# matteosantama/dantzig

Measured on AMD Instinct MI355X. Metric: simplex_iterations_per_sec, higher is better.
Workload: dtype f64

## Files before the change

### dantzig_amd/_ffi.py

```python
from __future__ import annotations

import ctypes as C
import os

import numpy as np

_HERE = os.path.dirname(os.path.abspath(__file__))
LIB_PATH = os.path.join(_HERE, "libdantzig_amd.so")

OPTIMAL, UNBOUNDED, INFEASIBLE, ITER_LIMIT, SINGULAR, PANIC, RUNNING, NEAR_TIE, NODE_LIMIT = range(9)
E_DEVICE, E_ARG, E_NOMEM = -1, -2, -3
STRICT, FAST, AUTO = 0, 1, 2
PRICE_AUTO, PRICE_SEQ, PRICE_WAVE, PRICE_TREE = 0, 1, 2, 3
STEP_PRIMAL, STEP_DUAL = 0, 1
NEAR_TIE_COUNT, NEAR_TIE_STOP = 0, 1
(K_STATUS, K_FTRAN, K_RATIO, K_BTRAN, K_PRICE, K_UPDATE, K_BASIS_UPDATE, K_LU, K_XCHG1, K_XCHG2,
 K_COUNT) = range(11)
KERNEL_CLASSES = ["status", "ftran", "ratio", "btran", "price", "update", "basis_update", "lu",
                  "exchange1", "exchange2"]

EXPORTS = [
    "dzg_abi_version", "dzg_status_str", "dzg_last_error", "dzg_device_count",
    "dzg_opts_default", "dzg_solver_create", "dzg_solver_run", "dzg_solver_result",
    "dzg_solver_destroy", "dzg_core_solve", "dzg_model_solve", "dzg_build_standard_form",
    "dzg_kernel_lu_solve", "dzg_kernel_neg_t_dot", "dzg_kernel_first_pivot",
    "dzg_kernel_second_pivot", "dzg_gen_dense_lp", "dzg_gen_sparse_lp", "dzg_merge_candidates",
    "dzg_shard_record_doubles", "dzg_shard_phase1", "dzg_shard_phase2", "dzg_shard_phase3",
    "dzg_solver_poll", "dzg_solver_set_budget", "dzg_comm_unique_id", "dzg_shard_comm_init",
    "dzg_shard_run", "dzg_shard_run_lockstep", "dzg_solver_stream", "dzg_solver_refactor",
    "dzg_gen_dense_lp_block", "dzg_solver_set_profile", "dzg_kernel_neg_t_dot_csc",
    "dzg_shard_comm_size", "dzg_solver_upload_columns", "dzg_debug_hold_cus", "dzg_debug_hold_wait",
    "dzg_core_solve_full_csc", "dzg_debug_live_lists", "dzg_debug_rl_listed",
    "dzg_debug_basis_inverse", "dzg_batch_solve", "dzg_model_solve_batch", "dzg_mip_opts_default",
    "dzg_mip_solve", "dzg_mip_last_warm_stats", "dzg_debug_cand_reduce", "dzg_debug_chain_instance",
    "dzg_debug_chain_price_counts", "dzg_debug_wk_mismatch", "dzg_debug_chain_price_rule",
    "dzg_solver_duals", "dzg_batch_solve_duals", "dzg_model_solve_duals",
    "dzg_model_solve_batch_duals", "dzg_model_map_duals",
    "dzg_solver_ranging", "dzg_batch_solve_ranging", "dzg_model_solve_ranging",
    "dzg_model_solve_batch_ranging",
    "dzg_solver_ray", "dzg_batch_solve_rays", "dzg_model_solve_rays", "dzg_model_solve_batch_rays",
    "dzg_model_map_ray",
    "dzg_batch_solve_fast", "dzg_model_solve_batch_fast", "dzg_debug_batch_fast_inverse",
    "dzg_solver_reoptimize",
    "dzg_solver_extend", "dzg_solver_dims", "dzg_debug_matrix", "dzg_debug_matrix_rows",
    "dzg_debug_extend_ms",
    "dzg_solver_remove",
    "dzg_batch_solve_from", "dzg_debug_batch_restart_ms",
]

BATCH_MAX_ROWS = 128
DUALS_FRESH, DUALS_CARRIED = 1, 2
DUALS_SOURCE_NAMES = {DUALS_FRESH: "fresh", DUALS_CARRIED: "carried"}
RAY_PRIMAL, RAY_FARKAS = 1, 2


class Lp(C.Structure):
    _fields_ = [
        ("m", C.c_int64), ("n", C.c_int64), ("n_struct", C.c_int64),
        ("a", C.c_void_p), ("lda", C.c_int64), ("var_col", C.c_void_p),
        ("c", C.c_void_p), ("constant", C.c_double),
        ("basis", C.c_void_p), ("nonbasis", C.c_void_p), ("x", C.c_void_p), ("z", C.c_void_p),
        ("col_ptr", C.c_void_p), ("row_idx", C.c_void_p), ("val", C.c_void_p),
        ("xbar", C.c_void_p), ("zbar", C.c_void_p),
    ]


class Opts(C.Structure):
    _fields_ = [
        ("numerics", C.c_int32), ("price_kernel", C.c_int32), ("device", C.c_int32),
        ("auto_strict_rows", C.c_int32), ("max_iter", C.c_int64), ("epsilon", C.c_double),
        ("log_capacity", C.c_int64), ("poll_interval", C.c_int32), ("profile", C.c_int32),
        ("col_begin", C.c_int64), ("col_end", C.c_int64), ("rank", C.c_int32),
        ("world", C.c_int32), ("stream", C.c_void_p), ("refactor_interval", C.c_int64),
        ("a_is_block", C.c_int32), ("near_tie_action", C.c_int32),
        ("replicate_matrix", C.c_int32), ("auto_restart_rows", C.c_int32), ("tie_tol", C.c_double),
        ("seven_launches", C.c_int32), ("auto_strict_budget_s", C.c_int32),
        ("shard_rows", C.c_int32), ("reserved0", C.c_int32),
    ]


class Pivot(C.Structure):
    _fields_ = [("kind", C.c_int32), ("reserved", C.c_int32), ("entering", C.c_int64),
                ("leaving", C.c_int64), ("mu", C.c_double)]


class Result(C.Structure):
    _fields_ = [
        ("status", C.c_int32), ("numerics_used", C.c_int32), ("iterations", C.c_int64),
# ... 133 lines not shown
def lib() -> C.CDLL:
    global _lib
    if _lib is None:
        if not os.path.exists(LIB_PATH):
            raise DantzigAmdError(
                f"{LIB_PATH} is missing: build the HIP engine first "
                "(python -m dantzig_amd._build). dantzig_amd has no CPU fallback.")
        _lib = C.CDLL(LIB_PATH)
        _lib.dzg_status_str.restype = C.c_char_p
        _lib.dzg_last_error.restype = C.c_char_p
        _lib.dzg_merge_candidates.restype = C.c_int64
        _lib.dzg_solver_destroy.restype = None
        _lib.dzg_opts_default.restype = None
        _lib.dzg_gen_dense_lp.argtypes = [C.c_uint64, C.c_int64, C.c_int64, C.c_void_p, C.c_int64,
                                          C.c_void_p, C.c_void_p]
        _lib.dzg_gen_dense_lp_block.argtypes = [C.c_uint64, C.c_int64, C.c_int64, C.c_int64,
                                                C.c_int64, C.c_void_p, C.c_int64, C.c_void_p,
                                                C.c_void_p]
        _lib.dzg_solver_run.argtypes = [C.c_void_p, C.c_int64]
        _lib.dzg_solver_result.argtypes = [C.c_void_p, C.c_void_p]
        _lib.dzg_solver_destroy.argtypes = [C.c_void_p]
        _lib.dzg_shard_record_doubles.restype = C.c_int64
        _lib.dzg_shard_record_doubles.argtypes = [C.c_void_p]
        _lib.dzg_shard_phase1.argtypes = [C.c_void_p, C.c_void_p]
        _lib.dzg_shard_phase2.argtypes = [C.c_void_p, C.c_void_p, C.c_void_p]
        _lib.dzg_shard_phase3.argtypes = [C.c_void_p, C.c_void_p]
        _lib.dzg_solver_poll.argtypes = [C.c_void_p, C.c_void_p, C.c_void_p]
        _lib.dzg_solver_set_budget.argtypes = [C.c_void_p, C.c_int64]
        _lib.dzg_comm_unique_id.argtypes = [C.c_void_p]
        _lib.dzg_shard_comm_init.argtypes = [C.c_void_p, C.c_void_p]
        _lib.dzg_shard_run.argtypes = [C.c_void_p, C.c_int64]
        _lib.dzg_shard_comm_size.argtypes = [C.c_void_p]
        _lib.dzg_shard_run_lockstep.argtypes = [C.c_void_p, C.c_int32, C.c_int64]
        _lib.dzg_solver_stream.restype = C.c_void_p
        _lib.dzg_solver_stream.argtypes = [C.c_void_p]
        _lib.dzg_solver_refactor.argtypes = [C.c_void_p]
        _lib.dzg_solver_set_profile.argtypes = [C.c_void_p, C.c_int32]
        _lib.dzg_core_solve_full_csc.argtypes = [C.c_int64, C.c_int64, C.c_void_p, C.c_void_p,
                                                 C.c_void_p, C.c_void_p, C.c_double, C.c_void_p,
                                                 C.c_void_p, C.c_void_p, C.c_void_p, C.c_void_p,
                                                 C.c_void_p]
        _lib.dzg_debug_hold_cus.argtypes = [C.c_int32, C.c_int32, C.c_double]
        _lib.dzg_debug_live_lists.restype = C.c_int64
        _lib.dzg_debug_live_lists.argtypes = [C.c_void_p, C.c_void_p]
        _lib.dzg_debug_basis_inverse.restype = C.c_int
        _lib.dzg_debug_basis_inverse.argtypes = [C.c_void_p, C.c_int64, C.c_int64, C.c_void_p, C.c_void_p]
        _lib.dzg_debug_cand_reduce.restype = C.c_int
        _lib.dzg_debug_cand_reduce.argtypes = [C.c_int32, C.c_int32, C.c_int64, C.c_void_p, C.c_void_p,
                                               C.c_void_p, C.c_void_p, C.c_void_p, C.c_void_p, C.c_void_p]
        _lib.dzg_debug_chain_instance.restype = C.c_int
        _lib.dzg_debug_chain_instance.argtypes = [C.c_int32] * 7
        _lib.dzg_debug_chain_price_counts.argtypes = [C.c_void_p, C.c_void_p]
        _lib.dzg_debug_wk_mismatch.argtypes = [C.c_void_p, C.c_int32, C.c_void_p]
        _lib.dzg_debug_chain_price_rule.restype = C.c_int
        _lib.dzg_debug_chain_price_rule.argtypes = [C.c_int32, C.c_int32, C.c_int32, C.c_int32, C.c_int64,
                                                    C.c_int32, C.c_int32]
        _lib.dzg_batch_solve.argtypes = [C.c_void_p, C.c_int64, C.c_void_p, C.c_int64, C.c_void_p]
        _lib.dzg_model_solve_batch.argtypes = [C.c_void_p, C.c_int64, C.c_void_p, C.c_void_p]
        _lib.dzg_batch_solve_fast.argtypes = [C.c_void_p, C.c_int64, C.c_void_p, C.c_int64, C.c_int64,
                                              C.c_void_p]
        _lib.dzg_model_solve_batch_fast.argtypes = [C.c_void_p, C.c_int64, C.c_void_p, C.c_void_p]
        _lib.dzg_debug_batch_fast_inverse.restype = C.c_int
        _lib.dzg_debug_batch_fast_inverse.argtypes = [C.c_void_p, C.c_int64, C.c_void_p, C.c_int64, C.c_int64,
                                                      C.c_void_p, C.c_void_p]
        _lib.dzg_solver_duals.argtypes = [C.c_void_p, C.c_void_p]
        _lib.dzg_batch_solve_duals.argtypes = [C.c_void_p, C.c_int64, C.c_void_p, C.c_int64, C.c_void_p,
                                               C.c_void_p]
        _lib.dzg_model_solve_duals.argtypes = [C.c_void_p, C.c_void_p, C.c_void_p, C.c_void_p]
        _lib.dzg_model_solve_batch_duals.argtypes = [C.c_void_p, C.c_int64, C.c_void_p, C.c_void_p,
                                                     C.c_void_p]
        _lib.dzg_model_map_duals.argtypes = [C.c_void_p, C.c_void_p, C.c_int64, C.c_void_p]
        _lib.dzg_solver_ranging.argtypes = [C.c_void_p, C.c_void_p, C.c_void_p, C.c_void_p]
        _lib.dzg_batch_solve_ranging.argtypes = [C.c_void_p, C.c_int64, C.c_void_p, C.c_int64, C.c_void_p,
                                                 C.c_void_p, C.c_void_p, C.c_void_p]
        _lib.dzg_model_solve_ranging.argtypes = [C.c_void_p, C.c_void_p, C.c_void_p, C.c_void_p, C.c_void_p,
                                                 C.c_void_p]
        _lib.dzg_model_solve_batch_ranging.argtypes = [C.c_void_p, C.c_int64, C.c_void_p, C.c_void_p,
                                                       C.c_void_p, C.c_void_p, C.c_void_p]
        _lib.dzg_solver_ray.argtypes = [C.c_void_p, C.c_void_p]
        _lib.dzg_batch_solve_rays.argtypes = [C.c_void_p, C.c_int64, C.c_void_p, C.c_int64, C.c_void_p,
                                              C.c_void_p, C.c_void_p]
        _lib.dzg_model_solve_rays.argtypes = [C.c_void_p, C.c_void_p, C.c_void_p, C.c_void_p, C.c_void_p]
        _lib.dzg_model_solve_batch_rays.argtypes = [C.c_void_p, C.c_int64, C.c_void_p, C.c_void_p,
                                                    C.c_void_p, C.c_void_p]
        _lib.dzg_model_map_ray.argtypes = [C.c_void_p, C.c_int32, C.c_void_p, C.c_void_p, C.c_int64,
                                           C.c_int64, C.c_void_p]
        _lib.dzg_solver_reoptimize.argtypes = [C.c_void_p, C.c_void_p]
        _lib.dzg_solver_extend.argtypes = [C.c_void_p, C.c_void_p]
        _lib.dzg_solver_remove.argtypes = [C.c_void_p, C.c_void_p, C.c_void_p, C.c_void_p]
        _lib.dzg_solver_dims.argtypes = [C.c_void_p, C.c_void_p, C.c_void_p, C.c_void_p]
        _lib.dzg_batch_solve_from.argtypes = [C.c_void_p, C.c_void_p, C.c_int64, C.c_void_p, C.c_int64,
                                              C.c_void_p, C.c_void_p]
        _lib.dzg_debug_batch_restart_ms.restype = C.c_double
        _lib.dzg_debug_batch_restart_ms.argtypes = []
        _lib.dzg_debug_matrix.argtypes = [C.c_void_p, C.c_int64, C.c_int64, C.c_void_p, C.c_int64]
        _lib.dzg_debug_matrix_rows.restype = C.c_int64
        _lib.dzg_debug_matrix_rows.argtypes = [C.c_void_p, C.c_int64, C.c_int64, C.c_void_p, C.c_int64]
        _lib.dzg_debug_extend_ms.argtypes = [C.c_void_p, C.c_void_p]
        _lib.dzg_mip_opts_default.restype = None
        _lib.dzg_mip_opts_default.argtypes = [C.c_void_p]
        _lib.dzg_mip_solve.argtypes = [C.c_void_p, C.c_void_p, C.c_void_p, C.c_void_p, C.c_void_p]
        _lib.dzg_mip_last_warm_stats.restype = None
        _lib.dzg_mip_last_warm_stats.argtypes = [C.c_void_p]
        _lib.dzg_solver_upload_columns.argtypes = [C.c_void_p, C.c_int64, C.c_int64, C.c_void_p,
                                                   C.c_int64]
    return _lib
# ... 127 lines not shown
```

### dantzig_amd/core.py

```python
from __future__ import annotations

import ctypes as C
from dataclasses import dataclass, field

import numpy as np

from . import _ffi
from ._ffi import (AUTO, FAST, STRICT, PRICE_AUTO, PRICE_SEQ, PRICE_WAVE, PRICE_TREE,
                   STEP_DUAL,
                   STEP_PRIMAL, NEAR_TIE_COUNT, NEAR_TIE_STOP, DantzigAmdError, f64, i64, ptr)

STATUS_NAMES = {0: "optimal", 1: "unbounded", 2: "infeasible", 3: "iter_limit", 4: "singular",
                5: "panic", 6: "running", 7: "near_tie"}


@dataclass
class CoreLP:
    a: np.ndarray | None
    c: np.ndarray
    basis: np.ndarray
    nonbasis: np.ndarray
    x: np.ndarray
    z: np.ndarray
    var_col: np.ndarray | None = None
# ... 451 lines not shown
        row_mask, col_mask = np.zeros(m, bool), np.zeros(ns, bool)
        row_mask[-1 - in_basis[in_basis < 0]] = True
        col_mask[out_of_basis[out_of_basis >= 0]] = True
        return row_mask, col_mask

    def remove(self, rows=None, cols=None) -> tuple[np.ndarray, np.ndarray]:
        if self._lp.a is None or self._lp.block is not None:
            raise NotImplementedError("remove is not supported on CSC storage or sharded solvers")
        drop_row, drop_col = _remove_lists(self._lp.m, self._lp.n_struct, rows, cols)
        lp2, _, _ = reduced_lp(self._at_current_basis(), rows, cols)
        r, c = np.flatnonzero(drop_row).astype(np.int64), np.flatnonzero(drop_col).astype(np.int64)
        var_map, row_map = np.zeros(self._lp.n, np.int64), np.zeros(self._lp.m, np.int64)
        rem = _ffi.Remove(len(r), ptr(r) if len(r) else None, len(c), ptr(c) if len(c) else None)
        _ffi.check_extend(_ffi.lib().dzg_solver_remove(self._h, C.byref(rem), ptr(var_map), ptr(row_map)),
                          "dzg_solver_remove")
        self._lp = lp2
        return var_map, row_map

    def dims(self) -> tuple[int, int, int]:
        v = [C.c_int64(0), C.c_int64(0), C.c_int64(0)]
        _ffi.check(_ffi.lib().dzg_solver_dims(self._h, *(C.byref(x) for x in v)), "dzg_solver_dims")
        return tuple(int(x.value) for x in v)

    def debug_matrix(self) -> np.ndarray:
        m, _, ns = self.dims()
        out = np.zeros((max(ns, 1), max(m, 1)))
        _ffi.check(_ffi.lib().dzg_debug_matrix(self._h, 0, ns, ptr(out), max(m, 1)), "dzg_debug_matrix")
        return out[:ns, :m].T.copy()

    def debug_matrix_rows(self) -> np.ndarray | None:
        m, _, ns = self.dims()
        out = np.zeros((max(m, 1), max(ns, 1)))
        got = _ffi.lib().dzg_debug_matrix_rows(self._h, 0, m, ptr(out), max(ns, 1))
        _ffi.check(int(got), "dzg_debug_matrix_rows")
        return out[:m, :ns].copy() if got == m and m > 0 else None

    def debug_extend_ms(self) -> tuple[float, float, float]:
        ms = np.zeros(3)
        _ffi.check(_ffi.lib().dzg_debug_extend_ms(self._h, ptr(ms)), "dzg_debug_extend_ms")
        return tuple(float(x) for x in ms)

    def debug_inverse(self, row0: int, row1: int) -> tuple[np.ndarray, dict]:
        m = self._lp.m
        out = np.zeros((max(int(row1) - int(row0), 0), m))
        info = np.zeros(4, np.int64)
        _ffi.check(_ffi.lib().dzg_debug_basis_inverse(self._h, int(row0), int(row1), ptr(out), ptr(info)),
                   "dzg_debug_basis_inverse")
        return out, dict(k=int(info[0]), neta=int(info[1]), rows=(int(info[2]), int(info[3])))

    def debug_chain_price_counts(self) -> tuple[int, int]:
        counts = np.zeros(2, np.int64)
        _ffi.check(_ffi.lib().dzg_debug_chain_price_counts(self._h, ptr(counts)), "dzg_debug_chain_price_counts")
        return int(counts[0]), int(counts[1])

    def debug_wk_mismatch(self, clear_valid: bool = False) -> tuple[int, bool]:
        info = np.zeros(2, np.int64)
        _ffi.check(_ffi.lib().dzg_debug_wk_mismatch(self._h, int(bool(clear_valid)), ptr(info)),
                   "dzg_debug_wk_mismatch")
        return int(info[0]), bool(info[1])

    def close(self) -> None:
        if self._h:
            _ffi.lib().dzg_solver_destroy(self._h)
            self._h = C.c_void_p(None)

    def __enter__(self):
        return self

    def __exit__(self, *exc):
        self.close()

    def __del__(self):
        try:
            self.close()
        except Exception:
            pass


def solve(lp: CoreLP, log: bool = True, **opts) -> CoreResult:
    with Solver(lp, **opts) as s:
        s.run(0)
        return s.result(log=log)


def core_solve(lp: CoreLP, log_cap: int = 1 << 20, **opts) -> CoreResult:
    with Solver.__new__(Solver)._prepare(lp, opts) as s:
        m, q = lp.m, lp.n - lp.m
        basis, nonbasis = np.zeros(max(m, 1), np.int64), np.zeros(max(q, 1), np.int64)
        x, xbar = np.zeros(max(m, 1)), np.zeros(max(m, 1))
        z, zbar = np.zeros(max(q, 1)), np.zeros(max(q, 1))
        buf = (_ffi.Pivot * max(log_cap, 1))()
        margins = np.full(max(log_cap, 1), np.inf)
        r = _ffi.Result()
        r.basis, r.nonbasis, r.x, r.xbar = ptr(basis), ptr(nonbasis), ptr(x), ptr(xbar)
        r.z, r.zbar = ptr(z), ptr(zbar)
        r.log, r.log_cap, r.margins = C.cast(buf, C.c_void_p), log_cap, ptr(margins)
        rc = _ffi.lib().dzg_core_solve(C.byref(s._c_lp), C.byref(s._opts), C.byref(r))
        _ffi.check(rc, "dzg_core_solve")
        cnt = int(min(r.iterations, log_cap))
        arr = np.ctypeslib.as_array(buf)[:cnt]
        pivots = list(zip(arr["kind"].tolist(), arr["entering"].tolist(),
                          arr["leaving"].tolist(), arr["mu"].tolist()))
        return CoreResult(
            status=STATUS_NAMES.get(r.status, str(r.status)), status_code=r.status,
            numerics="strict" if r.numerics_used == STRICT else "fast",
            iterations=int(r.iterations), objective=float(r.objective),
# ... 380 lines not shown
```

### dantzig_amd/csrc/engine.hip

```cpp
#include <dlfcn.h>

#include <chrono>
#include <cstdio>
#include <cstdlib>
#include <cstring>
#include <limits>
#include <string>
#include <utility>
#include <algorithm>
#include <vector>

#include "common.h"
#include "duals.h"
#include "ranging.h"
#include "rays.h"

static thread_local std::string g_err;

static int fail(int code, const std::string &msg)
{
    g_err = msg;
    return code;
}

// ... 320 lines not shown
static int successor_fill_matrix(dzg_solver *s, const SuccessorSrc &src);

static double ms_since(std::chrono::steady_clock::time_point t0)
{
    return std::chrono::duration<double, std::milli>(std::chrono::steady_clock::now() - t0).count();
}

static int solver_create(const dzg_lp *lp, const dzg_opts *opts_in, dzg_solver **out, const SuccessorSrc *src)
{
    if (!out) return fail(DZG_E_ARG, "out is NULL");
    *out = nullptr;
    std::string why;
    if (!validate(lp, why, src != nullptr)) return fail(DZG_E_ARG, "invalid dzg_lp: " + why);
    dzg_opts o;
    if (opts_in) o = *opts_in; else dzg_opts_default(&o);
    if (o.max_iter <= 0) o.max_iter = 10000000;
    if (o.poll_interval <= 0) o.poll_interval = 32;
    if (o.epsilon == 0.0) o.epsilon = 1e-12;
    if (o.auto_strict_rows <= 0) o.auto_strict_rows = 192;
    if (o.tie_tol == 0.0) o.tie_tol = 1e-11;

    int ndev = 0;
    if (hipGetDeviceCount(&ndev) != hipSuccess || ndev <= 0)
        return fail(DZG_E_DEVICE, "no HIP device visible: dantzig_amd has no CPU path");
    if (o.device < 0 || o.device >= ndev) return fail(DZG_E_ARG, "opts.device out of range");
    HIP_OK(hipSetDevice(o.device));

    dzg_solver *s = new dzg_solver();
    s->opts = o;
    struct Guard { dzg_solver *s; ~Guard() { if (s) dzg_solver_destroy(s); } } guard{s};
    if (o.stream) {
        s->st = (hipStream_t)o.stream;
        s->own_stream = false;
    } else {
        HIP_OK(hipStreamCreate(&s->st));
    }
    HIP_OK(hipHostMalloc((void **)&s->h_ctl, sizeof(DzgCtl)));

    DzgDev &d = s->d;
    const int m = (int)lp->m, n = (int)lp->n, ns = (int)lp->n_struct, q = n - m;
    d.m = m; d.n = n; d.ns = ns; d.q = q;
    d.lda = ((long long)m + 15) / 16 * 16 + (m >= 2048 ? 272 : 0);
    if (d.lda == 0) d.lda = 16;
    d.eps = o.epsilon;
    d.ftran_variant = -1;
    if (const char *fv = std::getenv("DZG_FTRAN_VARIANT")) d.ftran_variant = std::atoi(fv);
    {
        const double kk = 384e6 / (8.0 * (double)(lp->m > 0 ? lp->m : 1));
        d.ftran_nt_k = kk > 2e9 ? 2000000000 : (int)kk;
        if (d.ftran_nt_k < 513) d.ftran_nt_k = 513;
    }
    d.beta_split = 1;
    if (const char *bs = std::getenv("DZG_CHAIN_BETA_SPLIT")) d.beta_split = bs[0] != '0';
    d.fold_k = 0x7fffffff;
    if (const char *fk = std::getenv("DZG_CHAIN_FOLD_K")) d.fold_k = std::atoi(fk);
    d.world = o.world > 1 ? o.world : 1;
    d.rank = d.world > 1 ? o.rank : 0;
    d.col0 = 0;
    d.col1 = ns;
    if (d.world > 1) {
        if (o.rank < 0 || o.rank >= o.world || o.col_begin < 0 || o.col_end > ns ||
            o.col_begin > o.col_end)
            return fail(DZG_E_ARG, "opts.rank / col_begin / col_end");
        d.col0 = (int)o.col_begin;
        d.col1 = (int)o.col_end;
    }
    const int nloc = d.col1 - d.col0;
    d.repl = (d.world > 1 && o.replicate_matrix && lp->a) ? 1 : 0;
    d.xstride = d.repl ? 8 : 8 + ((long long)m + 7) / 8 * 8;
    const double *a_host = !lp->a ? nullptr
                           : (o.a_is_block && d.world > 1) ? lp->a
                                                           : lp->a + (size_t)d.col0 * (size_t)lp->lda;

    d.csc = (ns > 0 && !lp->a && !src) ? 1 : 0;
    d.rs = 0;
    d.rs_r0 = 0;
    d.rs_r1 = m;
    d.rs_mcol = 0;
    if (o.shard_rows && d.world > 1) {
        if (d.csc) return fail(DZG_E_ARG, "opts.shard_rows needs a dense matrix");
        if (o.price_kernel != DZG_PRICE_AUTO && o.price_kernel != DZG_PRICE_TREE)
            return fail(DZG_E_ARG, "opts.shard_rows prices with the AUTO / TREE kernels (every rank "
                                   "re-derives dz of the entering column in their summation order)");
        d.rs = 1;
        s->rs_slice = (int)((((long long)m + d.world - 1) / d.world + 15) / 16 * 16);
        if (s->rs_slice < 16) s->rs_slice = 16;
        const long long r0 = (long long)d.rank * s->rs_slice;
        d.rs_r0 = (int)(r0 < m ? r0 : m);
        d.rs_r1 = (int)(r0 + s->rs_slice < m ? r0 + s->rs_slice : m);
        d.rs_mcol = d.repl ? 0 : ((long long)m + 15) / 16 * 16;
        s->xstride_max = DZG_RS_COL + d.rs_mcol + ((long long)m + 2 + 15) / 16 * 16;
        d.xstride = s->xstride_max;
    }
    if (d.csc) {
        std::vector<long long> cp((size_t)nloc + 1, 0);
        std::vector<int> ri;
        std::vector<double> cv;
        for (int j = 0; j < nloc; ++j) {
            for (int64_t e = lp->col_ptr[d.col0 + j]; e < lp->col_ptr[d.col0 + j + 1]; ++e)
                if (lp->val[e] != 0.0) {
                    ri.push_back((int)lp->row_idx[e]);
                    cv.push_back(lp->val[e]);
                }
            cp[(size_t)j + 1] = (long long)ri.size();
        }
        long long *dcp; int *dri; double *dcv;
// ... 2924 lines not shown
    for (int64_t k = 0; k < ncols; ++k) {
        if (cols[k] >= n_struct || cols[k] < -m) return fail(DZG_E_ARG, "cols out of range");
        c32[(size_t)k] = (int)cols[k];
    }
    long long *dcp; int *dri, *dcols; double *dcv, *dv, *dout;
    HIP_OK(hipMalloc(&dcp, sizeof(long long) * cp.size()));
    HIP_OK(hipMalloc(&dri, sizeof(int) * (nnz + 1)));
    HIP_OK(hipMalloc(&dcv, sizeof(double) * (nnz + 1)));
    HIP_OK(hipMalloc(&dv, sizeof(double) * ((size_t)m + 2)));
    HIP_OK(hipMalloc(&dout, sizeof(double) * c32.size()));
    HIP_OK(hipMalloc(&dcols, sizeof(int) * c32.size()));
    HIP_OK(hipMemcpy(dcp, cp.data(), sizeof(long long) * cp.size(), hipMemcpyHostToDevice));
    if (nnz) {
        HIP_OK(hipMemcpy(dri, row_idx, sizeof(int) * nnz, hipMemcpyHostToDevice));
        HIP_OK(hipMemcpy(dcv, val, sizeof(double) * nnz, hipMemcpyHostToDevice));
    }
    HIP_OK(hipMemset(dv, 0, sizeof(double) * ((size_t)m + 2)));
    HIP_OK(hipMemcpy(dv, v, sizeof(double) * m, hipMemcpyHostToDevice));
    HIP_OK(hipMemcpy(dcols, c32.data(), sizeof(int) * c32.size(), hipMemcpyHostToDevice));
    dzg_launch_price_csc_raw(dcp, dri, dcv, dcols, (int)ncols, dv, dout, 0);
    HIP_OK(hipDeviceSynchronize());
    HIP_OK(hipGetLastError());
    if (ncols > 0) HIP_OK(hipMemcpy(out, dout, sizeof(double) * ncols, hipMemcpyDeviceToHost));
    hipFree(dcp); hipFree(dri); hipFree(dcv); hipFree(dv); hipFree(dout); hipFree(dcols);
    return 0;
}

extern "C" int dzg_kernel_first_pivot(int64_t len, const double *y, const double *ybar,
                                      int64_t *pos_out, int32_t device)
{
    if (len < 0 || !pos_out) return fail(DZG_E_ARG, "bad argument");
    if (dzg_device_count() <= 0) return fail(DZG_E_DEVICE, "no HIP device visible");
    HIP_OK(hipSetDevice(device));
    return dzg_run_first_pivot(len, y, ybar, pos_out);
}

extern "C" int dzg_kernel_second_pivot(int64_t len, double mu, const double *y, const double *ybar,
                                       const double *dy, int64_t *pos_out, int32_t device)
{
    if (len < 0 || !pos_out) return fail(DZG_E_ARG, "bad argument");
    if (dzg_device_count() <= 0) return fail(DZG_E_DEVICE, "no HIP device visible");
    HIP_OK(hipSetDevice(device));
    return dzg_run_second_pivot(len, mu, y, ybar, dy, pos_out);
}

extern "C" int dzg_debug_chain_price_counts(dzg_solver *s, int64_t counts[2])
{
    if (!s || !counts) return fail(DZG_E_ARG, "NULL argument");
    counts[0] = s->chain_fused;
    counts[1] = s->chain_unfused;
    return 0;
}

extern "C" int dzg_debug_chain_price_rule(int32_t m, int32_t grid, int32_t k_hint, int32_t tiles, int64_t q,
                                          int32_t small, int32_t timed)
{
    return dzg_chain_price_rule(m, grid, k_hint, tiles, q, small, timed);
}

extern "C" int dzg_debug_wk_mismatch(dzg_solver *s, int32_t clear_valid, int64_t info[2])
{
    if (!s || !info) return fail(DZG_E_ARG, "NULL argument");
    const DzgDev &d = s->d;
    if (!s->wk_buf) return fail(DZG_E_ARG, "wk mismatch: this solver keeps no compact copy of the eta rows");
    HIP_OK(hipSetDevice(s->opts.device));
    TRY(read_ctl(s));
    const int k = s->h_ctl->ncompact, neta = s->h_ctl->neta;
    if (k < 0 || k > d.m || neta < 0 || neta > DZG_RMAX)
        return fail(DZG_E_DEVICE, "wk mismatch: control block out of range");
    info[1] = s->d.wk ? 1 : 0;
    dzg_launch_gather_wk(d, d.Wc, s->st);
    const size_t n = (size_t)d.ldw * DZG_RMAX;
    std::vector<double> kept(n), fresh(n);
    HIP_OK(hipMemcpyAsync(kept.data(), s->wk_buf, sizeof(double) * n, hipMemcpyDeviceToHost, s->st));
    HIP_OK(hipMemcpyAsync(fresh.data(), d.Wc, sizeof(double) * n, hipMemcpyDeviceToHost, s->st));
    HIP_OK(hipStreamSynchronize(s->st));
    HIP_OK(hipGetLastError());
    int64_t bad = 0;
    for (int t = 0; t < neta; ++t)
        for (int c = 0; c < k; ++c)
            bad += std::memcmp(&kept[(size_t)t * d.ldw + c], &fresh[(size_t)t * d.ldw + c], sizeof(double)) != 0;
    info[0] = bad;
    if (clear_valid) s->d.wk = nullptr;
    return 0;
}
```

### dantzig_amd/csrc/k_chain.hip

```cpp
#include <chrono>
#include "common.h"
#include "fast_decide.h"
#include "fast_rows.h"
#include "price_small.h"

#include "chain_barrier.h"


#define CH_NW (CH_THREADS / 64)
#define CH_MAXP 16

template <bool NARROW>
__device__ __forceinline__ bool chain_wide(int k)
{
    if constexpr (NARROW)
        return false;
    else
        return k > 512;
}
template <bool NOFOLD>
__device__ __forceinline__ int chain_fold_on(int fold)
{
    if constexpr (NOFOLD)
        return 0;
// ... 154 lines not shown
__device__ __forceinline__ const double *chain_col(const DzgDev &d, int code,
                                                   const double *__restrict__ xrecv, int w_rec)
{
    if (code < 0) return nullptr;
    if (SHARD && d.xstride > 8) return xrecv + (long long)w_rec * d.xstride + 8;
    return d.A + (long long)(code - d.col0) * d.lda;
}

#define CH_BETA_WAVE 3
__device__ __forceinline__ void chain_beta_item(const DzgDev &d, int item, int code,
                                                const double *__restrict__ a)
{
    const int t = item >> 2, w = item & 3;
    const double *wt = d.W + (long long)t * d.ldw;
    double s;
    if (code < 0) {
        if (w != 0) return;
        s = wt[-1 - code];
    } else {
        s = fast_beta_wave(wt, a, d.m, w);
    }
    if ((threadIdx.x & 63) == 0) st_sc1(d.beta_part + item, s);
}
__device__ __forceinline__ void chain_beta(const DzgDev &d, int neta, int code,
                                           const double *__restrict__ a)
{
    const int wave = threadIdx.x >> 6;
    if (!d.beta_split) {
        for (int b = blockIdx.x; b < neta; b += gridDim.x)
            if (wave < 4) chain_beta_item(d, 4 * b + wave, code, a);
        return;
    }
    int turn = CH_BETA_WAVE;
    for (int item = blockIdx.x; item < 4 * neta; item += gridDim.x) {
        if (wave == turn) chain_beta_item(d, item, code, a);
        turn = turn + 1 < CH_NW ? turn + 1 : 0;
    }
}
__device__ __forceinline__ void chain_beta_published()
{
    __builtin_amdgcn_s_waitcnt(0);
}
__device__ __forceinline__ void chain_beta_fetch(const DzgDev &d, int neta, int code, double *s_beta)
{
    const int tid = threadIdx.x;
    if (tid < 4 * R_) {
        const double s0 = tid < 4 * neta ? ld_sc1(d.beta_part + tid) : 0.0;
        const double s1 = __shfl_down(s0, 1, DZG_WAVE);
        const double s2 = __shfl_down(s0, 2, DZG_WAVE);
        const double s3 = __shfl_down(s0, 3, DZG_WAVE);
        const int t = tid >> 2;
        if ((tid & 3) == 0) s_beta[t] = t < neta ? (code < 0 ? s0 : fast_beta_fold(s0, s1, s2, s3)) : 0.0;
    }
}

template <int LPR, int MAXP>
__device__ __forceinline__ void chain_dot_head(const DzgDev &d, int r0, int r1, int k,
                                               const double *s_ag, double (&accs)[MAXP])
{
    constexpr int RPW = 64 / LPR;
    const int lane = threadIdx.x & 63, wave = threadIdx.x >> 6;
    const int sub = lane % LPR, grp = lane / LPR;
    const int k2 = (k + 1) & ~1;
    const int variant = d.ftran_variant >= 0 ? d.ftran_variant : (k >= d.ftran_nt_k ? 2 : 0);
    if (LPR == 64 && variant == 1) {
#pragma unroll
        for (int pass = 0; pass < MAXP; ++pass) {
            const int i = r0 + (pass * CH_NW + wave) * RPW + grp;
            accs[pass] = fast_gemv_row_head<LPR, 1>(i < r1 ? i : d.m, d.m, k2, d.binv, d.ldb, s_ag, sub);
        }
        return;
    }
    if (LPR == 64 && variant == 2) {
#pragma unroll
        for (int pass = 0; pass < MAXP; ++pass) {
            const int i = r0 + (pass * CH_NW + wave) * RPW + grp;
            accs[pass] = fast_gemv_row_head<LPR, 2>(i < r1 ? i : d.m, d.m, k2, d.binv, d.ldb, s_ag, sub);
        }
        return;
    }
#pragma unroll
    for (int pass = 0; pass < MAXP; ++pass) {
        const int i = r0 + (pass * CH_NW + wave) * RPW + grp;
        accs[pass] = fast_gemv_row_head<LPR>(i < r1 ? i : d.m, d.m, k2, d.binv, d.ldb, s_ag, sub);
    }
}

template <int LPR, int MAXP>
__device__ __forceinline__ void chain_dot_tail(const DzgDev &d, int r0, int r1, int k, int neta,
                                               const double *s_ag, const double *s_beta,
                                               const double (&accs)[MAXP], double *s_dx)
{
    constexpr int RPW = 64 / LPR;
    const int lane = threadIdx.x & 63, wave = threadIdx.x >> 6;
    const int sub = lane % LPR, grp = lane / LPR;
    const int k2 = (k + 1) & ~1;
    const int npass = (r1 - r0 + CH_NW * RPW - 1) / (CH_NW * RPW);
#pragma unroll
    for (int pass = 0; pass < MAXP; ++pass) {
        if (pass < npass) {
            const int i = r0 + (pass * CH_NW + wave) * RPW + grp;
            const int ii = i < r1 ? i : d.m;
            const double acc = fast_gemv_row_tail<LPR>(accs[pass], ii, d.m, neta, d.U, d.ldw, s_beta, sub);
            if (ii < d.m && sub == 0) s_dx[i - r0] = acc;
        }
    }
// ... 68 lines not shown
    DzgCtl c = *ctl;
    if (c.status != DZG_RUNNING) return;
    unsigned long long gen = c.bar_gen;
    const int neta = c.neta, k = c.ncompact;
    const int dr0 = tid < k ? d.drow[tid] : -1;
    const int dr1 = tid + CH_THREADS < k ? d.drow[tid + CH_THREADS] : -1;
    if (wave < 2 && !(SHARD && wave == 0)) {
        chain_spec_pin(ts, sp);
        const unsigned long long t_site = ts.now();
        DzgCand2 w = chain_spec_reduce(sp, c.fp_count, lane);
        ts.pin(w);
        ts.site(DZG_SITE_PRE_FIRST, t_site);
        if (lane == 0) chain_put(s_c, wave, w);
    }
    __syncthreads();
    const DzgCand2 cj = SHARD ? cj_rec : chain_get(s_c, 0), ci = chain_get(s_c, 1);
    int kind;
    double mu;
    const unsigned long long t_status = ts.now();
    if (!fast_status(ctl, c, lead, cj, ci, d.eps, m, SHARD, kind, &mu)) return;
    ts.pin(mu);
    ts.site(DZG_SITE_PRE_STATUS, t_status);
    const int slot = kind == DZG_STEP_PRIMAL ? 0 : 1;
    ts.mark(slot);
    if (k > CH_AGCAP || c.fp_count > 256 || (NARROW && k > 512)) {
        if (lead) ctl->status = DZG_PANIC;
        return;
    }
    if (PRICE != 0 && (k >= d.rows_T || k >= CH_THREADS - CHP_COL0 || r1 - r0 > CHP_COL0 ||
                       tiles > nwg || (long long)tiles * CH_THREADS < d.q || !d.wk)) {
        if (lead) ctl->status = DZG_PANIC;
        return;
    }
    if (lead) {
        ctl->neta_cur = neta;
        ctl->k_cur = k;
    }
    int p;
    if (kind == DZG_STEP_PRIMAL) {
        const int epos = cj.k;
        const int code = d.nbcode[epos];
        double zr = 0.0, zbr = 0.0;
        if (lead) {
            zr = d.z[epos];
            zbr = d.zbar[epos];
        }
        const double *a = chain_col<SHARD>(d, code, xrecv, w_rec);
        const bool has_unit = has_row && bcode_i < 0;
        double unit_i = 0.0;
        if (has_unit) unit_i = code >= 0 ? a[-1 - bcode_i] : (code == bcode_i ? 1.0 : 0.0);
        int edslot = -1;
        if (lead && code < 0) edslot = d.dslot[-1 - code];
        chain_stage_ag(s_ag, k, code, a, d.drow, dr0, dr1);
        chain_beta(d, neta, code, a);
        ts.mark(slot);
        if (lead) {
            ctl->enter_code = code;
            ctl->zr = zr;
            ctl->zbar_r = zbr;
            ctl->enter_dslot = edslot;
            if (SHARD) ctl->enter_src = w_rec;
        }
        __syncthreads();
        double accs[MAXP];
        if (chain_wide<NARROW>(k))
            chain_dot_head<64>(d, r0, r1, k, s_ag, accs);
        else
            chain_dot_head<16>(d, r0, r1, k, s_ag, accs);
        chain_beta_published();
        ts.mark(slot);
        if (!chain_barrier(ctl, bar, gen)) return;
        ts.mark(slot);
        chain_beta_fetch(d, neta, code, s_beta);
        __syncthreads();
        if (chain_wide<NARROW>(k))
            chain_dot_tail<64>(d, r0, r1, k, neta, s_ag, s_beta, accs, s_dx);
        else
            chain_dot_tail<16>(d, r0, r1, k, neta, s_ag, s_beta, accs, s_dx);
        __syncthreads();
        DzgCand2 best = dzg_cand2_none();
        if (has_row) {
            double dxi = s_dx[tid];
            if (has_unit) dxi += unit_i;
            d.dx[row] = dxi;
            const double scaled = mu * xbar_i;
            const double den = x_i + scaled;
            DzgCand2 cnd;
            cnd.r = dzg_div(dxi, den);
            cnd.k = row;
            cnd.h = -__builtin_inf();
            if (cnd.r > 0.0) best = dzg_better2(best, cnd);
            if (dzg_noise_zero(den, x_i, scaled, c.tau)) best.h = __builtin_inf();
        }
        ts.pin(best);
        const unsigned long long t_rowbest = ts.now();
        best = chain_best(best, r1 - r0);
        ts.pin(best);
        ts.site(DZG_SITE_PRE_ROWBEST, t_rowbest);
        if (tid == 0) {
            st_sc1(d.rx_r + blockIdx.x, best.r);
            st_sc1(d.rx_k + blockIdx.x, best.k);
            st_sc1(d.rx_h + blockIdx.x, best.h);
        }
        ts.mark(slot);
        if (!chain_barrier(ctl, bar, gen)) return;
        ts.mark(slot);
        const unsigned long long t_sc1 = ts.now();
        if (wave == 0) {
            const DzgCand2 w = chain_reduce_sc1(d.rx_r, d.rx_k, d.rx_h, nwg, lane);
            if (lane == 0) chain_put(s_c, 0, w);
        }
        __syncthreads();
        DzgCand2 cw = chain_get(s_c, 0);
        ts.pin(cw);
        ts.site(DZG_SITE_PRE_SC1, t_sc1);
        if (!fast_ratio_outcome(ctl, c, lead, cw, DZG_UNBOUNDED)) {
            if (lead) ctl->bar_gen = gen;
            return;
        }
        p = cw.k;
        if (lead) ctl->leave_pos = p;
        ts.mark(slot);
    } else {
        p = ci.k;
    }
    const int lcode = d.bcode[p];
// ... 717 lines not shown
```

### include/dantzig_amd.h

```cpp
#ifndef DANTZIG_AMD_H
#define DANTZIG_AMD_H

#include <stdint.h>

#ifdef __cplusplus
extern "C" {
#endif

#define DZG_ABI_VERSION 4

typedef enum {
    DZG_OPTIMAL = 0,
    DZG_UNBOUNDED = 1,
    DZG_INFEASIBLE = 2,
    DZG_ITER_LIMIT = 3,
    DZG_SINGULAR = 4,
    DZG_PANIC = 5,
    DZG_RUNNING = 6,
    DZG_NEAR_TIE = 7,
    DZG_NODE_LIMIT = 8,
    DZG_E_DEVICE = -1,
    DZG_E_ARG = -2,
    DZG_E_NOMEM = -3
} dzg_status;
// ... 391 lines not shown
int dzg_kernel_second_pivot(int64_t len, double mu, const double *y, const double *ybar,
                            const double *dy, int64_t *pos_out, int32_t device);


int dzg_gen_sparse_lp(uint64_t seed, int64_t m, int64_t n_struct, int64_t per_col,
                      int64_t *col_ptr, int32_t *row_idx, double *val, double *b, double *c);

int dzg_gen_dense_lp(uint64_t seed, int64_t m, int64_t n_struct, double *a, int64_t lda,
                     double *b, double *c);

int dzg_gen_dense_lp_block(uint64_t seed, int64_t m, int64_t n_struct, int64_t col_begin,
                           int64_t col_end, double *a_block, int64_t lda, double *b, double *c);

typedef struct {
    double ratio;
    int64_t pos;
    double y, ybar, dy;
} dzg_candidate;

int64_t dzg_shard_record_doubles(const dzg_solver *s);
int dzg_shard_phase1(dzg_solver *s, double *send_dev);
int dzg_shard_phase2(dzg_solver *s, const double *recv_dev, double *send_dev);
int dzg_shard_phase3(dzg_solver *s, const double *recv_dev);
int dzg_comm_unique_id(void *unique_id_128);
int dzg_shard_comm_init(dzg_solver *s, const void *unique_id_128);
int dzg_shard_run(dzg_solver *s, int64_t max_new_iters);
int dzg_shard_comm_size(dzg_solver *s);
int dzg_shard_run_lockstep(dzg_solver **solvers, int32_t world, int64_t max_new_iters);
void *dzg_solver_stream(dzg_solver *s);
int dzg_solver_set_profile(dzg_solver *s, int32_t mask);
int dzg_solver_poll(dzg_solver *s, int32_t *status, int64_t *iterations);
int dzg_solver_set_budget(dzg_solver *s, int64_t max_new_iters);

int dzg_debug_hold_cus(int32_t device, int32_t workgroups, double seconds);
int dzg_debug_hold_wait(void);

int64_t dzg_debug_live_lists(dzg_solver *s, int64_t *entries);
int64_t dzg_debug_rl_listed(dzg_solver *s);
int dzg_debug_matrix(dzg_solver *s, int64_t col0, int64_t col1, double *out, int64_t ld_out);
int64_t dzg_debug_matrix_rows(dzg_solver *s, int64_t row0, int64_t row1, double *out, int64_t ld_out);
int dzg_debug_extend_ms(const dzg_solver *s, double ms[3]);
int dzg_debug_basis_inverse(dzg_solver *s, int64_t row0, int64_t row1, double *out, int64_t info[4]);
int dzg_debug_batch_fast_inverse(const dzg_lp *lps, int64_t count, const dzg_opts *opts, int64_t pivots,
                                 int64_t refactor_every, double *w_out, dzg_result *res);

int dzg_debug_cand_reduce(int32_t device, int32_t form, int64_t ncases, const double *r, const int32_t *k,
                          const double *h, const int32_t *count, double *out_r, int32_t *out_k,
                          double *out_h);

int dzg_debug_chain_instance(int32_t m, int32_t grid, int32_t k_bound, int32_t fold, int32_t nrz,
                             int32_t shard, int32_t post);

int dzg_debug_chain_price_counts(dzg_solver *s, int64_t counts[2]);
int dzg_debug_wk_mismatch(dzg_solver *s, int32_t clear_valid, int64_t info[2]);
int dzg_debug_chain_price_rule(int32_t m, int32_t grid, int32_t k_hint, int32_t tiles, int64_t q,
                               int32_t small, int32_t timed);

int64_t dzg_merge_candidates(const dzg_candidate *cands, int64_t count);

#ifdef __cplusplus
}
#endif
#endif
```

Baseline: 35350.

## Skip grid barrier when entering column's beta is computable locally

When the entering variable is a slack (code < 0) or no eta columns exist, and beta_split is 1, each block loads beta directly from W instead of computing partial betas and synchronizing across the grid. This removes one grid-wide barrier per simplex iteration in those cases. An env var can disable the skip (beta_split=2), and a debug entry point reports the barrier generation count. The risk is extra W loads per block and a possible correctness issue if the local load does not match the folded global result.

```diff
diff --git a/dantzig_amd/_ffi.py b/dantzig_amd/_ffi.py
--- a/dantzig_amd/_ffi.py
+++ b/dantzig_amd/_ffi.py
@@ -34,6 +34,7 @@
     "dzg_debug_basis_inverse", "dzg_batch_solve", "dzg_model_solve_batch", "dzg_mip_opts_default",
     "dzg_mip_solve", "dzg_mip_last_warm_stats", "dzg_debug_cand_reduce", "dzg_debug_chain_instance",
     "dzg_debug_chain_price_counts", "dzg_debug_wk_mismatch", "dzg_debug_chain_price_rule",
+    "dzg_debug_chain_barriers",
     "dzg_solver_duals", "dzg_batch_solve_duals", "dzg_model_solve_duals",
     "dzg_model_solve_batch_duals", "dzg_model_map_duals",
     "dzg_solver_ranging", "dzg_batch_solve_ranging", "dzg_model_solve_ranging",
@@ -273,6 +274,7 @@
         _lib.dzg_debug_chain_instance.argtypes = [C.c_int32] * 7
         _lib.dzg_debug_chain_price_counts.argtypes = [C.c_void_p, C.c_void_p]
         _lib.dzg_debug_wk_mismatch.argtypes = [C.c_void_p, C.c_int32, C.c_void_p]
+        _lib.dzg_debug_chain_barriers.argtypes = [C.c_void_p, C.c_void_p]
         _lib.dzg_debug_chain_price_rule.restype = C.c_int
         _lib.dzg_debug_chain_price_rule.argtypes = [C.c_int32, C.c_int32, C.c_int32, C.c_int32, C.c_int64,
                                                     C.c_int32, C.c_int32]
diff --git a/dantzig_amd/core.py b/dantzig_amd/core.py
--- a/dantzig_amd/core.py
+++ b/dantzig_amd/core.py
@@ -527,6 +527,11 @@
         counts = np.zeros(2, np.int64)
         _ffi.check(_ffi.lib().dzg_debug_chain_price_counts(self._h, ptr(counts)), "dzg_debug_chain_price_counts")
         return int(counts[0]), int(counts[1])
+
+    def debug_chain_barriers(self) -> int:
+        passed = np.zeros(1, np.int64)
+        _ffi.check(_ffi.lib().dzg_debug_chain_barriers(self._h, ptr(passed)), "dzg_debug_chain_barriers")
+        return int(passed[0])
 
     def debug_wk_mismatch(self, clear_valid: bool = False) -> tuple[int, bool]:
         info = np.zeros(2, np.int64)
diff --git a/dantzig_amd/csrc/engine.hip b/dantzig_amd/csrc/engine.hip
--- a/dantzig_amd/csrc/engine.hip
+++ b/dantzig_amd/csrc/engine.hip
@@ -396,6 +396,8 @@
     }
     d.beta_split = 1;
     if (const char *bs = std::getenv("DZG_CHAIN_BETA_SPLIT")) d.beta_split = bs[0] != '0';
+    if (const char *sb = std::getenv("DZG_CHAIN_SLACK_BARRIER"))
+        if (sb[0] == '1' && d.beta_split) d.beta_split = 2;
     d.fold_k = 0x7fffffff;
     if (const char *fk = std::getenv("DZG_CHAIN_FOLD_K")) d.fold_k = std::atoi(fk);
     d.world = o.world > 1 ? o.world : 1;
@@ -3426,6 +3428,15 @@
     return 0;
 }
 
+extern "C" int dzg_debug_chain_barriers(dzg_solver *s, int64_t *passed)
+{
+    if (!s || !passed) return fail(DZG_E_ARG, "NULL argument");
+    HIP_OK(hipSetDevice(s->opts.device));
+    TRY(read_ctl(s));
+    *passed = (int64_t)s->h_ctl->bar_gen;
+    return 0;
+}
+
 extern "C" int dzg_debug_chain_price_rule(int32_t m, int32_t grid, int32_t k_hint, int32_t tiles, int64_t q,
                                           int32_t small, int32_t timed)
 {
diff --git a/dantzig_amd/csrc/k_chain.hip b/dantzig_amd/csrc/k_chain.hip
--- a/dantzig_amd/csrc/k_chain.hip
+++ b/dantzig_amd/csrc/k_chain.hip
@@ -230,6 +230,23 @@
         const int t = tid >> 2;
         if ((tid & 3) == 0) s_beta[t] = t < neta ? (code < 0 ? s0 : fast_beta_fold(s0, s1, s2, s3)) : 0.0;
     }
+}
+
+__device__ __forceinline__ bool chain_beta_is_local(const DzgDev &d, int neta, int code)
+{
+    return (code < 0 || neta == 0) && d.beta_split == 1;
+}
+__device__ __forceinline__ double chain_beta_local_load(const DzgDev &d, int neta, int code)
+{
+    const int tid = threadIdx.x, t = tid & 63;
+    if ((tid >> 6) != CH_BETA_WAVE || t >= neta || code >= 0) return 0.0;
+    return d.W[(long long)t * d.ldw + (-1 - code)];
+}
+__device__ __forceinline__ void chain_beta_local_put(double b, double *s_beta)
+{
+    static_assert(R_ <= 64, "one wave holds beta");
+    const int tid = threadIdx.x, t = tid & 63;
+    if ((tid >> 6) == CH_BETA_WAVE && t < R_) s_beta[t] = b;
 }
 
 template <int LPR, int MAXP>
@@ -404,7 +421,12 @@
         int edslot = -1;
         if (lead && code < 0) edslot = d.dslot[-1 - code];
         chain_stage_ag(s_ag, k, code, a, d.drow, dr0, dr1);
-        chain_beta(d, neta, code, a);
+        const bool beta_local = !SHARD && __builtin_amdgcn_readfirstlane((int)chain_beta_is_local(d, neta, code));
+        double beta_l = 0.0;
+        if (beta_local)
+            beta_l = chain_beta_local_load(d, neta, code);
+        else
+            chain_beta(d, neta, code, a);
         ts.mark(slot);
         if (lead) {
             ctl->enter_code = code;
@@ -419,11 +441,17 @@
             chain_dot_head<64>(d, r0, r1, k, s_ag, accs);
         else
             chain_dot_head<16>(d, r0, r1, k, s_ag, accs);
-        chain_beta_published();
-        ts.mark(slot);
-        if (!chain_barrier(ctl, bar, gen)) return;
-        ts.mark(slot);
-        chain_beta_fetch(d, neta, code, s_beta);
+        if (!SHARD && __builtin_amdgcn_readfirstlane((int)chain_beta_is_local(d, neta, code))) {
+            ts.mark(slot);
+            ts.mark(slot);
+            chain_beta_local_put(beta_l, s_beta);
+        } else {
+            chain_beta_published();
+            ts.mark(slot);
+            if (!chain_barrier(ctl, bar, gen)) return;
+            ts.mark(slot);
+            chain_beta_fetch(d, neta, code, s_beta);
+        }
         __syncthreads();
         if (chain_wide<NARROW>(k))
             chain_dot_tail<64>(d, r0, r1, k, neta, s_ag, s_beta, accs, s_dx);
diff --git a/include/dantzig_amd.h b/include/dantzig_amd.h
--- a/include/dantzig_amd.h
+++ b/include/dantzig_amd.h
@@ -467,6 +467,7 @@
                              int32_t shard, int32_t post);
 
 int dzg_debug_chain_price_counts(dzg_solver *s, int64_t counts[2]);
+int dzg_debug_chain_barriers(dzg_solver *s, int64_t *passed);
 int dzg_debug_wk_mismatch(dzg_solver *s, int32_t clear_valid, int64_t info[2]);
 int dzg_debug_chain_price_rule(int32_t m, int32_t grid, int32_t k_hint, int32_t tiles, int64_t q,
                                int32_t small, int32_t timed);
```

New measurement: 35770, median of 5. 1.01x the previous value.
